# electrum/presto

Hardware: AMD Instinct MI355X
Metric: rows/s through operator pipeline, TPC-H Q1+Q6 SF100, 1/2/4/8 GPUs vs CPU ref (higher is better)
Workload: dtype f64

## Files before the change

presto_amd/csrc/fused_codegen.cpp:

```cpp
#include "decimal_host.hpp"
#include "fused_codegen.hpp"
#include "scan_kernels.hpp"

namespace pa {
namespace fused {

int range_entry_words(const Spec& s, const std::vector<ChannelLayout>& layout)
{
    int words = 1;
    for (int c = 0; c < s.n_in; c++) {
        if (!s.used_channel[c]) continue;
        words += 1 + (layout[c].type == PA_VARCHAR ? 1 : 0) + (layout[c].nullable ? 1 : 0);
    }
    return words;
}

static std::vector<ChannelLayout> extended_layout(const Spec& s, const std::vector<ChannelLayout>& layout)
{
    std::vector<ChannelLayout> ext(layout.begin(), layout.begin() + s.n_in);
    if (s.join) {
        for (size_t v = 0; v < s.join->build_cols.size(); v++) {
            ChannelLayout cl;
            cl.type = s.join->build_types[v];
            cl.nullable = (size_t)s.n_in + v < layout.size() ? layout[(size_t)s.n_in + v].nullable : true;
// ... 123 lines not shown
{
    if ((int)word_terms.size() <= w) word_terms.resize(w + 1);
    word_terms[w].push_back(term);
}

void FusedGen::group_keys()
{
    const std::vector<int>& gp = brow ? s.join->brow_group_proj : s.group_proj;
    std::ostringstream& kinner = brow ? key_os : inner;
    for (size_t gi = 0; gi < gp.size(); gi++) {
        const GenValue& kv = key_value(gp[gi]);
        const OwnedExpr& pe = s.proj[gp[gi]];
        KeyPart part;
        part.type = kv.type;
        std::string value;
        switch (kv.type) {
            case PA_BIGINT:
            case PA_DECIMAL:
                part.bits = 64;
                value = "(u64)" + kv.v;
                break;
            case PA_INTEGER:
            case PA_DATE:
                part.bits = 32;
                value = "(u64)(u32)(i32)" + kv.v;
                break;
            case PA_REAL:
                part.bits = 32;
                value = "(u64)pa_real_key_bits(" + kv.v + ")";
                break;
            case PA_BOOLEAN:
                part.bits = 1;
                value = "(" + kv.v + " ? 1ULL : 0ULL)";
                break;
            case PA_DOUBLE:
                part.bits = 64;
                value = "((" + kv.v + " == 0.0) ? 0ULL : ((" + kv.v + " != " + kv.v + ") ? 0x7ff8000000000000ULL : (u64)__double_as_longlong(" +
                        kv.v + ")))";
                break;
            case PA_VARCHAR: {
                int ch = pe.is_input_ref() ? pe.node(pe.root).channel : -1;
                if (ch >= 0 && ch < s.n_in && s.short_bound[ch] > 0) {
                    part.bound = s.short_bound[ch];
                    part.bits = 8 * part.bound + 4;
                    value = "(cs" + std::to_string(ch) + " | ((u64)" + kv.len + " << " + std::to_string(8 * part.bound) + "))";
                }
                else {
                    part.bits = 128;
                }
                break;
            }
            default:
                throw Error(PA_ERR_NOT_SUPPORTED, "group key type not supported on device");
        }
        std::string guard = kv.nullable() ? "(" + kv.n + ") ? 0ULL : " : "";
        if (part.bits == 128) {
            int sh;
            part.word = packer.place(64, &sh);
            int w2 = packer.place(64, &sh);
            PA_REQUIRE(w2 == part.word + 1, PA_ERR_NOT_SUPPORTED, "internal: long VARCHAR key words not adjacent");
            std::string id = "ks" + std::to_string(gi);
            kinner << "u64 " << id << "a = 0, " << id << "b = 0;\n";
            kinner << "if (" << (kv.nullable() ? "!" + kv.n : "true") << ") {\n";
            kinner << "  if (" << kv.len << " > 15) pa_raise(a.err, -3);\n";
            kinner << "  for (i32 b = 0; b < " << kv.len << " && b < 15; b++) {\n";
            kinner << "    if (b < 8) " << id << "a |= (u64)" << kv.v << "[b] << (8 * b); else " << id << "b |= (u64)" << kv.v
                  << "[b] << (8 * (b - 8));\n  }\n";
            kinner << "  " << id << "b |= (u64)" << kv.len << " << 56;\n}\n";
            add_term(part.word, id + "a");
            add_term(part.word + 1, id + "b");
        }
        else {
            part.word = packer.place(part.bits, &part.shift);
            add_term(part.word, "((" + guard + value + ") << " + std::to_string(part.shift) + ")");
        }
        if (kv.nullable()) {
            part.null_word = packer.place(1, &part.null_shift);
            add_term(part.null_word, "((" + kv.n + ") ? " + std::to_string(1ULL << part.null_shift) + "ULL : 0ULL)");
        }
        k.keys.push_back(part);
    }
    k.w = (int)packer.used.size();
    PA_REQUIRE(k.w <= 8, PA_ERR_NOT_SUPPORTED, "group key wider than 8 words");
}

int FusedGen::word(int kind, const std::string& cond, const std::string& val, const std::string& key)
{
    auto it = word_index.find(key);
    if (it != word_index.end()) return it->second;
    words.push_back({kind, cond, val});
    word_index[key] = (int)words.size() - 1;
    return (int)words.size() - 1;
}

std::string FusedGen::minmax_image(const GenValue& x, bool is_min)
{
    std::string img;
    switch (x.type) {
        case PA_BIGINT:
        case PA_INTEGER:
        case PA_DECIMAL:
        case PA_DATE: img = "pa_img_i64((i64)" + x.v + ")"; break;
        case PA_DOUBLE: img = "pa_img_f64(" + x.v + ")"; break;
        case PA_REAL: img = "pa_img_f64((double)" + x.v + ")"; break;
        case PA_BOOLEAN: img = "(" + x.v + " ? 1ULL : 0ULL)"; break;
        case PA_VARCHAR: img = "pa_img_str7(" + x.v + ", " + x.len + ", a.err)"; break;
        default: throw Error(PA_ERR_NOT_SUPPORTED, "min/max input type not supported on device");
    }
    return is_min ? "(~" + img + ")" : img;
}

std::string FusedGen::wtype(int w) const
{
    return words[w].kind == W_SUMF ? "double" : (words[w].kind == W_MAXU ? "u64" : "i64");
}

void FusedGen::accumulator_words()
{
    for (const auto& ag : s.aggs) {
        if (s.step == PA_STEP_FINAL) {
            const GenValue& c = proj_value(ag.input_channel);
            std::string ch = std::to_string(ag.input_channel);
            std::string ccond = c.nullable() ? "(!" + c.n + ")" : "true";
            int cw = word(W_CNT, ccond, c.v, "fcnt|" + ch);
            int vw = -1;
            if (ag.fn == PA_AGG_SUM || ag.fn == PA_AGG_AVG) {
                const GenValue& v = proj_value(ag.input_channel + 1);
                std::string vcond = v.nullable() ? "(" + ccond + " && !" + v.n + ")" : ccond;
                if (v.type == PA_LONG_DECIMAL) {
                    const int limbs = decimal_limbs_for_bits(128);
                    for (int l = 0; l < limbs; l++) {
                        const int w = word(W_SUMI, vcond, "pa_dec_limb(" + v.v + ", " + std::to_string(l) + ", " + std::to_string(limbs - 1) + ")", "fdec" + std::to_string(l) + "|" + ch);
                        if (l == 0) vw = w;
                        PA_REQUIRE(w == vw + l, PA_ERR_NOT_SUPPORTED, "internal: the limb words of a DECIMAL sum are not adjacent");
                    }
                    k.agg_words.emplace_back(cw, vw);
                    k.agg_limbs.resize(k.agg_words.size(), 0);
                    k.agg_limbs.back() = limbs;
                    continue;
                }
                vw = word(v.type == PA_DOUBLE ? W_SUMF : W_SUMI, vcond, v.v, "fsum|" + ch);
            }
            else if (ag.fn == PA_AGG_MIN || ag.fn == PA_AGG_MAX) {
                const GenValue& v = proj_value(ag.input_channel + 1);
                std::string vcond = v.nullable() ? "(" + ccond + " && !" + v.n + ")" : ccond;
                vw = word(W_MAXU, vcond, minmax_image(v, ag.fn == PA_AGG_MIN), std::string(ag.fn == PA_AGG_MIN ? "fmin|" : "fmax|") + ch);
            }
            k.agg_words.emplace_back(cw, vw);
            continue;
        }
        std::string cond = "true", ckey = "m" + std::to_string(ag.mask_channel);
        if (ag.mask_channel >= 0) {
            const GenValue& m = proj_value(ag.mask_channel);
            PA_REQUIRE(m.type == PA_BOOLEAN, PA_ERR_INVALID_ARGUMENT, "mask channel must be BOOLEAN");
            cond = m.nullable() ? "(!" + m.n + " && " + m.v + ")" : "(" + m.v + ")";
        }
        if (ag.fn == PA_AGG_COUNT_STAR) {
            k.agg_words.emplace_back(word(W_CNT, cond, "1", "cnt|*|" + ckey), -1);
            continue;
        }
        const GenValue& x = proj_value(ag.input_channel);
        std::string xkey = s.proj[ag.input_channel].fingerprint();
        std::string ccond = cond, cntkey = "cnt|*|" + ckey;
        if (x.nullable()) {
            ccond = "(" + cond + " && !" + x.n + ")";
            cntkey = "cnt|" + xkey + "|" + ckey;
        }
        const bool implicit_count = s.step == PA_STEP_SINGLE && !s.group_proj.empty() && ag.mask_channel < 0 && !x.nullable() &&
                                    (ag.fn == PA_AGG_SUM || ag.fn == PA_AGG_MIN || ag.fn == PA_AGG_MAX);
        int cw = implicit_count ? -1 : word(W_CNT, ccond, "1", cntkey);
        int vw = -1;
        if ((ag.fn == PA_AGG_SUM || ag.fn == PA_AGG_AVG) && (x.type == PA_DECIMAL || x.type == PA_LONG_DECIMAL)) {
            const int limbs = decimal_limbs_for_bits(std::min(x.type == PA_DECIMAL ? 64 : 128, decimal_bits_for_precision(PA_DECIMAL_PRECISION(x.param))));
            for (int l = 0; l < limbs; l++) {
                const int w = word(W_SUMI, ccond, "pa_dec_limb((i128)" + x.v + ", " + std::to_string(l) + ", " + std::to_string(limbs - 1) + ")",
                                   "dec" + std::to_string(l) + "/" + std::to_string(limbs) + "|" + xkey + "|" + ckey);
                if (l == 0) vw = w;
                PA_REQUIRE(w == vw + l, PA_ERR_NOT_SUPPORTED, "internal: the limb words of a DECIMAL sum are not adjacent");
            }
            k.agg_words.emplace_back(cw, vw);
            k.agg_limbs.resize(k.agg_words.size(), 0);
            k.agg_limbs.back() = limbs;
            continue;
        }
        if (ag.fn == PA_AGG_SUM && x.type != PA_DOUBLE && x.type != PA_REAL) {
            vw = word(W_SUMI, ccond, x.v, "sumi|" + xkey + "|" + ckey);
        }
        else if (ag.fn == PA_AGG_SUM || ag.fn == PA_AGG_AVG) {
            std::string v = x.type == PA_DOUBLE ? x.v : "((double)" + x.v + ")";
            vw = word(W_SUMF, ccond, v, std::string("sumf|") + (x.type == PA_DOUBLE ? "d|" : "i|") + xkey + "|" + ckey);
        }
        else if (ag.fn == PA_AGG_MIN || ag.fn == PA_AGG_MAX) {
            vw = word(W_MAXU, ccond, minmax_image(x, ag.fn == PA_AGG_MIN), std::string(ag.fn == PA_AGG_MIN ? "min|" : "max|") + xkey + "|" + ckey);
        }
        k.agg_words.emplace_back(cw, vw);
    }
    k.nw = (int)words.size();
    k.agg_limbs.resize(k.agg_words.size(), 0);
    PA_REQUIRE(k.nw > 0 || k.w > 0, PA_ERR_INVALID_ARGUMENT, "aggregation without aggregates and keys");
    if (k.nw == 0) {
        words.push_back({W_CNT, "true", "1"});
        k.nw = 1;
    }
    for (const auto& w : words) k.word_kind.push_back(w.kind);
}

void FusedGen::state_layout_id()
{
    std::vector<std::string> names(words.size(), "rows");
    for (const auto& kv : word_index) names[(size_t)kv.second] = kv.first;
    std::ostringstream id;
    for (const KeyPart& kp : k.keys) {
        id << kp.type << ',' << kp.word << ',' << kp.shift << ',' << kp.bits << ',' << kp.bound << ',' << kp.null_word << ',' << kp.null_shift << ';';
    }
    id << '#';
    for (size_t w = 0; w < words.size(); w++) id << words[w].kind << ':' << names[w] << ';';
    k.layout_id = id.str();
}

void FusedGen::row_function(const std::string& name)
{
    if (s.join) {
        probe_row_frames();
    }
    else {
        src << "__device__ __forceinline__ void " << name << "(const PaFusedArgs& a, PaAcc& acc, const bool live, const i32 row" << row_params(ri, layout) << ")\n{\n";
    }
    src << body.str();
    for (int w = 0; w < k.nw; w++) {
        src << "bool u" << w << " = false; " << (words[w].kind == W_SUMF ? "double" : (words[w].kind == W_MAXU ? "u64" : "i64")) << " x" << w << " = 0;\n";
    }
    if (k.w > 0) src << "u64 key[PA_KW];\n#pragma unroll\nfor (int i = 0; i < PA_KW; i++) key[i] = 0;\n";
    src << "if (sel) {\n" << build_loads.str() << inner.str();
    for (int w = 0; w < k.nw; w++) src << "u" << w << " = " << words[w].cond << "; x" << w << " = " << words[w].val << ";\n";
    if (brow) {
        src << "key[0] = (u64)(u32)jb;\n";
    }
    else {
        for (int i = 0; i < k.w; i++) {
            src << "key[" << i << "] = ";
            for (size_t t = 0; t < word_terms[i].size(); t++) src << (t ? " | " : "") << word_terms[i][t];
            src << ";\n";
        }
    }
    src << "}\n";
    if (variant == V_HASH) hash_accumulate_row();
    else if (variant == V_GLOBAL) global_accumulate_row();
    else if (variant == V_LDS) lds_accumulate_row();
    else if (brow) brow_accumulate_row();
    else table_accumulate_row();
    src << "}\n\n";
}

void FusedGen::emit_quad(const std::string (&args)[4])
{
    if (s.join) {
        probe_quad(args);
        return;
    }
    for (int r = 0; r < 4; r++) src << "        pa_row(a, acc, true, (i32)(4 * q + " << r << ")" << args[r] << ");\n";
}

void FusedGen::emit_kernel(const std::string& name, int mode)
{
    std::string occupancy;
    if (brow) {
        if (const char* e = getenv("PRESTO_AMD_BROW_WAVES")) occupancy = " __attribute__((amdgpu_waves_per_eu(" + std::to_string(atoi(e)) + ")))";
    }
    src << "extern \"C\" __global__ __launch_bounds__(" << B << ")" << occupancy << " void PA_K(" << name << ")(PaFusedArgs a)\n{\n";
    if (variant == V_GLOBAL) global_kernel_begin();
    else if (variant == V_LDS) lds_kernel_begin();
    else if (variant == V_LDSP) ldsp_kernel_begin();
    else if (variant == V_LDSH) ldsh_kernel_begin();
    else if (variant == V_HASH) hash_kernel_begin();
    else if (brow) brow_kernel_begin();
    else gt_kernel_begin();
    if (mode != 2 && mode != 3) emit_prologue(ri, layout, src);
    if (mode == 3) {
        ranges_loop();
    }
    else if (variant == V_GLOBAL) {
        global_thread_ids();
    }
    else {
        src << "    const i64 t = (i64)blockIdx.x * " << B << " + threadIdx.x, T = (i64)gridDim.x * " << B << ";\n";
    }
    if (mode == 3) {
    }
    else if (mode == 1) lds_head_loop();
    else if (mode == 2) lds_tail_loop();
    else if (variant == V_HASH) hash_tile_loop();
    else page_loop();
    if (variant == V_LDSP) ldsp_partition_loop();
    if (variant == V_GT || variant == V_LDSH) list_loops();
    if (variant == V_LDSH) ldsh_kernel_end();
    if (brow) brow_kernel_end();
    if (gt_like || brow || lds_table) table_counter_flush();
    if (variant == V_GLOBAL) global_kernel_end();
    else if (variant == V_LDS) lds_kernel_end();
    src << "}\n\n";
}

void FusedGen::ranges_loop()
{
    ColumnNames rn;
    rn.ranged = true;
    const int rw = range_entry_words(s, layout);
    src << "    const u32 bsw = (gridDim.x & 7u) == 0u ? (blockIdx.x & 7u) * (gridDim.x >> 3) + (blockIdx.x >> 3) : blockIdx.x;\n"
           "    for (i64 ri = bsw; ri < a.n_ranges; ri += gridDim.x) {\n"
           "      const u64* RT = a.ranges + (u64)ri * " << rw << "ULL;\n";
    int at = 0;
    for (int c = 0; c < s.n_in; c++) {
        if (!ri.used[c]) continue;
        src << "      const void* const RV" << c << " = (const void*)RT[" << at++ << "];\n";
        if (layout[c].type == PA_VARCHAR) src << "      const i32* const RO" << c << " = (const i32*)RT[" << at++ << "];\n";
        if (layout[c].nullable) src << "      const u8* const RNL" << c << " = (const u8*)RT[" << at++ << "];\n";
    }
    src << "      const i64 RN = (i64)(RT[" << at << "] & 0xffffffffULL);\n"
           "      const bool rvec = (RT[" << at << "] >> 32) != 0ULL;\n";
    {
        std::ostringstream pro;
        emit_prologue(ri, layout, pro, rn);
        src << pro.str();
    }
    if (variant == V_LDS) src << "      const i64 nq = rvec ? (RN >> 8) << 6 : 0;\n";
    else src << "      const i64 nq = rvec ? RN >> 2 : 0;\n";
    src << "      for (i64 q = threadIdx.x; q < nq; q += " << B << ") {\n";
    std::string rargs[4];
    emit_vector_loads(ri, layout, src, rargs, rn);
    emit_quad(rargs);
    src << "      }\n";
    if (variant == V_LDS) {
        src << "      for (i64 rb = nq << 2; rb < RN; rb += 64) {\n        const bool live = rb + threadIdx.x < RN;\n"
               "        const i64 r = live ? rb + threadIdx.x : RN - 1;\n        pa_row(a, acc, live, (i32)r" << scalar_args(ri, layout, rn) << ");\n      }\n";
    }
    else {
        src << "      for (i64 r = (nq << 2) + threadIdx.x; r < RN; r += " << B << ") {\n        pa_row(a, acc, true, (i32)r" << scalar_args(ri, layout, rn) << ");\n      }\n";
    }
    src << "    }\n";
}

void FusedGen::page_loop()
{
    std::string args[4];
    src << "    const i64 nq = a.vec ? (a.n >> 2) : 0;\n";
    const std::string tail_rows = "    for (i64 r = (nq << 2) + t; r < a.n; r += T) {\n        pa_row(a, acc, true, (i32)r" + scalar_args(ri, layout) + ");" + flush + "\n    }\n";
    bool two_loops = false;
    if (staged) {
        staged_page_loop();
        src << tail_rows;
        return;
    }
    if (brow) {
        int level = 3;
        if (const char* e = getenv("PRESTO_AMD_BROW_PIPE")) level = atoi(e);
        std::vector<VectorVar> vars;
        const bool can = level > 0 && s.join && vector_load_vars(ri, layout, vars);
        if (can && level < 3) {
            brow_pipelined_loop(level);
            src << tail_rows;
            return;
        }
        if (can) {
            src << "    if (a.jrank) {\n";
            brow_pipelined_loop(level);
            src << "    } else {\n";
            two_loops = true;
        }
        brow_wave_loop_head();
    }
    else {
// ... 17 lines not shown
```

presto_amd/csrc/fused_codegen.hpp:

```cpp
#pragma once

#include <functional>
#include <map>
#include <sstream>
#include <string>
#include <vector>

#include "fused_plan.hpp"
#include "rowgen.hpp"

namespace pa {
namespace fused {

struct KeyPacker {
    std::vector<int> used;
    int place(int bits, int* shift)
    {
        for (size_t w = 0; w < used.size(); w++) {
            if (used[w] + bits <= 64) {
                *shift = used[w];
                used[w] += bits;
                return (int)w;
            }
        }
        used.push_back(bits);
        *shift = 0;
        return (int)used.size() - 1;
    }
};

struct WordDef {
    int kind;
    std::string cond;
    std::string val;
};

struct FusedGen {
    FusedGen(const Spec& spec, const std::vector<ChannelLayout>& page_layout, int requested_variant);
    KernelInfo run();

    const Spec& s;
    const std::vector<ChannelLayout>& layout;
    int variant;
    bool ranged;
    KernelInfo k;
    RowInputs ri;
    std::vector<ChannelLayout> ext;
    RowCodegen gen;
    std::ostringstream body;
    std::ostringstream pre;
    std::ostringstream inner;
    std::ostringstream key_os;
    std::ostringstream build_loads;
    std::ostringstream src;
    std::map<int, GenValue> pv, kpv;
    KeyPacker packer;
    std::vector<std::vector<std::string>> word_terms;
    std::vector<WordDef> words;
    std::map<std::string, int> word_index;
    bool brow = false, lds_table = false, gt_like = false;
    bool staged = false;
    std::string lazy_params, lazy_names;
    int B = 256;
    std::string flush;

    const GenValue& proj_value(int j);
    const GenValue& key_value(int j);
    void add_term(int word, const std::string& term);
    int word(int kind, const std::string& cond, const std::string& val, const std::string& key);
    std::string minmax_image(const GenValue& x, bool is_min);
    std::string wtype(int w) const;
    void row_filter();
    void group_keys();
    void accumulator_words();
    void state_layout_id();
    void row_function(const std::string& name = "pa_row");
    void emit_quad(const std::string (&args)[4]);
    void emit_kernel(const std::string& name, int mode);
    void ranges_loop();
    void page_loop();
    void table_counter_flush();

    void global_declarations();
    void global_accumulate_row();
    void global_kernel_begin();
    void global_thread_ids();
    void global_kernel_end();
    void staged_row_functions();
    void staged_page_loop();

    void lds_check_capacity();
    void lds_declarations();
    void lds_accumulate_row();
    void lds_kernel_begin();
    void lds_head_loop();
    void lds_tail_loop();
    void lds_kernel_end();

    void lds_table_size();
    void lds_table_declarations();
    void lds_table_accumulate_begin();
    void ldsh_kernel_begin();
    void ldsh_kernel_end();

    void hash_declarations();
    void hash_accumulate_row();
    void hash_kernel_begin();
    void hash_tile_loop();
    void ldsp_kernel_begin();
    void ldsp_partition_loop();

    void gt_declarations();
    void table_accumulate();
    void gt_run_combining();
    void table_accumulate_row();
    void gt_kernel_begin();
    void list_loops();

    void probe_filter_and_key(const std::string& sel);
    void probe_occupancy_word();
    void probe_build_loads();
    std::string lazy_assign(const std::string& suffix, const std::string& row);
    std::string lazy_declare(const std::string& suffix);
    void probe_row_frames();
    void probe_row_composition();
    void probe_quad(const std::string (&args)[4]);
    void brow_declarations();
    void brow_accumulate_row();
    void brow_kernel_begin();
    void brow_wave_loop_head();
    bool brow_pipelined_loop(int level);
    void brow_kernel_end();
    void brow_keys_kernel();
};

}
}
```

presto_amd/csrc/fused_plan.hpp:

```cpp
#pragma once

#include <map>
#include <memory>
#include <string>
#include <vector>

#include "exprgen.hpp"
#include "join_source.hpp"
#include "operator.hpp"

namespace pa {
namespace fused {

constexpr int kMaxChannels = 32;
constexpr int kMaxBuildChannels = 8;

struct FusedArgs {
    const void* v[kMaxChannels];
    const int32_t* o[kMaxChannels];
    const uint8_t* nl[kMaxChannels];
    int64_t n;
    int32_t vec;
    int32_t pad;
    uint64_t* slab;
// ... 18 lines not shown
    uint64_t* sub_tag;
    uint64_t* sub_keys;
    uint64_t* sub_words;
    int32_t* sub_count;
    const int64_t* part_first;
    const void* jslots;
    const uint64_t* jbits;
    int64_t jmin;
    uint64_t jrange;
    uint32_t jmask;
    int32_t jrows;
    uint32_t jwrap;
    uint32_t jpad;
    const void* bv[kMaxBuildChannels];
    const uint8_t* bn[kMaxBuildChannels];
    const void* jrank;
    const int32_t* jrank_rows;
    const uint64_t* ranges;
    int64_t n_ranges;
};

enum Variant { V_GLOBAL = 0, V_LDS = 1, V_GT = 2, V_LDSH = 3, V_HASH = 4, V_LDSP = 5, V_BROW = 6, V_GLOBAL_R = 7, V_LDS_R = 8, V_GLOBAL_S = 9 };
constexpr int kMaxStages = 4;
constexpr int64_t kRangeRows = 8192, kRangeRowsLds = 4096;
enum WordKind { W_CNT = 0, W_SUMF = 1, W_SUMI = 2, W_MAXU = 3 };

constexpr int kLdsSlots = 8;

struct KeyPart {
    int32_t type = PA_BIGINT;
    int word = 0;
    int shift = 0;
    int bits = 64;
    int bound = 0;
    int null_word = -1;
    int null_shift = 0;
};

struct JoinStage {
    std::shared_ptr<LookupSourceImpl> ls;
    int key_proj = -1;
    std::vector<int> build_cols;
    std::vector<int32_t> build_types;
    std::vector<int> brow_group_proj;
};

struct Spec {
    std::shared_ptr<JoinStage> join;
    std::vector<bool> lazy_channel;
    std::vector<int32_t> conjuncts;
    std::vector<int> conjunct_begin;
    std::vector<int> channel_stage;
    int n_stages = 0;
    int n_in = 0;
    std::vector<int32_t> in_types, in_params;
    bool has_filter = false;
    OwnedExpr filter;
    std::vector<OwnedExpr> proj;
    std::vector<int> group_proj;
    int hash_channel = -1;
    std::vector<pa_aggregate> aggs;
    int expected_groups = 0;
    int64_t max_partial_memory = 0;
    int step = PA_STEP_SINGLE;
    int output_mem = PA_MEM_HOST;
    std::vector<bool> used_channel;
    std::vector<int> short_bound;
    std::vector<bool> interned;
    std::vector<bool> ranked;
    bool any_ranked() const
    {
        for (bool r : ranked) if (r) return true;
        return false;
    }
    bool derived(int c) const { return interned[c] || ranked[c]; }
};

struct KernelInfo {
    std::string source, entry;
    int variant = V_GLOBAL;
    bool ranged = false;
    std::vector<int> stage_bytes;
    int nw = 0, w = 0, c = 0, block = 256;
    int lc = 0;
    int occ_word = -1;
    uint64_t occ_empty = 0;
    std::vector<int32_t> word_kind;
    std::vector<std::pair<int, int>> agg_words;
    std::vector<int> agg_limbs;
    std::vector<KeyPart> keys;
    std::string layout_id;
};

struct LayoutChange {};

OwnedExpr input_ref_expr(int32_t channel, int32_t type);
Spec make_spec(const pa_filter_project_desc& fp, const pa_hash_aggregation_desc& ag, const pa_lookup_join_desc* jd = nullptr,
               pa_lookup_source* bridge = nullptr);
Spec make_spec(const pa_fused_aggregation_desc* d);
void finalize_spec(Spec& s);
void plan_stages(Spec& s);

int range_entry_words(const Spec& s, const std::vector<ChannelLayout>& layout);
KernelInfo generate(const Spec& s, const std::vector<ChannelLayout>& layout, int variant);

}
}
```

presto_amd/csrc/fused_tier_lds.cpp:

```cpp
#include "decimal_host.hpp"
#include "fused_codegen.hpp"
#include "scan_kernels.hpp"

namespace pa {
namespace fused {

void FusedGen::lds_check_capacity()
{
    PA_REQUIRE((size_t)k.nw * kLdsSlots * 64 * 8 <= 64 * 1024, PA_ERR_NOT_SUPPORTED, "too many accumulator words for the LDS variant");
}

void FusedGen::lds_declarations()
{
    src << "__shared__ u64 pa_accw[PA_NW * PA_C * 64];\n";
    src << "struct PaAcc { u64 tk[PA_C][PA_KW]; int tcount; u32 lane; };\n";
}

void FusedGen::lds_accumulate_row()
{
    src << "int g = -1;\nif (sel) {\n#pragma unroll\n  for (int s = 0; s < PA_C; s++) {\n    bool eq = s < acc.tcount;\n#pragma unroll\n"
           "    for (int w = 0; w < PA_KW; w++) eq = eq && (key[w] == acc.tk[s][w]);\n    if (eq) g = s;\n  }\n}\n";
    src << "u64 miss = __ballot(sel && g < 0);\nwhile (miss != 0ULL) {\n  const int src_lane = __builtin_amdgcn_readfirstlane(__ffsll((long long)miss) - 1);\n"
           "  u64 nk[PA_KW];\n#pragma unroll\n  for (int w = 0; w < PA_KW; w++) nk[w] = pa_readlane_u64(key[w], src_lane);\n"
           "  const int slot = acc.tcount;\n  if (slot < PA_C) {\n#pragma unroll\n    for (int s = 0; s < PA_C; s++) {\n      if (s == slot) {\n#pragma unroll\n"
           "        for (int w = 0; w < PA_KW; w++) acc.tk[s][w] = nk[w];\n      }\n    }\n    acc.tcount = slot + 1;\n  } else {\n    acc.tcount = PA_C + 1;\n  }\n"
           "  bool mine = sel && g == -1;\n#pragma unroll\n  for (int w = 0; w < PA_KW; w++) mine = mine && (key[w] == nk[w]);\n"
           "  if (mine) g = slot < PA_C ? slot : -2;\n  miss = __ballot(sel && g == -1);\n}\n";
    src << "if (sel) {\n  if (g >= 0) {\n";
    for (int w = 0; w < k.nw; w++) {
        std::string idx = "pa_accw[(" + std::to_string(w) + " * PA_C + g) * 64 + acc.lane]";
        if (words[w].kind == W_SUMF) {
            src << "    if (u" << w << ") __hip_atomic_fetch_add((double*)&" << idx << ", x" << w << ", __ATOMIC_RELAXED, __HIP_MEMORY_SCOPE_WORKGROUP);\n";
        }
        else if (words[w].kind == W_SUMI) {
            src << "    if (u" << w << ") { i64* p = (i64*)&" << idx << "; *p = pa_add_exact(*p, x" << w << ", a.err); }\n";
        }
        else if (words[w].kind == W_MAXU) {
            src << "    if (u" << w << ") { u64* p = &" << idx << "; if (x" << w << " > *p) *p = x" << w << "; }\n";
        }
        else {
            src << "    if (u" << w << ") __hip_atomic_fetch_add(&" << idx << ", " << (words[w].val == "1" ? std::string("1ULL") : "(u64)x" + std::to_string(w))
                << ", __ATOMIC_RELAXED, __HIP_MEMORY_SCOPE_WORKGROUP);\n";
        }
    }
    src << "  }\n}\n";
}

void FusedGen::lds_kernel_begin()
{
    src << "    for (int i = threadIdx.x; i < PA_NW * PA_C * 64; i += 64) pa_accw[i] = 0ULL;\n";
    src << "    __syncthreads();\n";
    src << "    PaAcc acc; acc.tcount = 0; acc.lane = threadIdx.x;\n";
    src << "#pragma unroll\n    for (int s = 0; s < PA_C; s++) {\n#pragma unroll\n        for (int w = 0; w < PA_KW; w++) acc.tk[s][w] = 0ULL;\n    }\n";
}

void FusedGen::lds_head_loop()
{
    std::string args[4];
    src << "    const i64 nq = a.n >> 2;  // the host passes a multiple of 256 rows\n";
    src << "    for (i64 q = t; q < nq; q += T) {\n";
    emit_vector_loads(ri, layout, src, args);
    emit_quad(args);
    src << "    }\n";
}

void FusedGen::lds_tail_loop()
{
    src << "    for (i64 rb = (i64)blockIdx.x * 64; rb < a.n; rb += T) {\n        const bool live = rb + threadIdx.x < a.n;\n"
           "        const i64 r = live ? rb + threadIdx.x : a.n - 1;\n        pa_row(a, acc, live, (i32)r" << scalar_args(ri, layout) << ");\n    }\n";
}

void FusedGen::lds_kernel_end()
{
    src << "    __syncthreads();\n";
    src << "    if (acc.tcount > PA_C && threadIdx.x == 0) atomicAdd((unsigned long long*)a.overflow_rows, 1ULL);\n";
    src << "    const u64 E = (u64)gridDim.x * PA_C;\n";
    src << "#pragma unroll\n    for (int i = 0; i < PA_C; i++) {\n        u64* e = a.slab + (u64)blockIdx.x * PA_C + i;\n";
    src << "        const bool occ = i < acc.tcount;\n        if (threadIdx.x == 0) e[0] = occ ? 1ULL : 0ULL;\n        if (occ) {\n";
    src << "#pragma unroll\n            for (int w = 0; w < PA_KW; w++) { if (threadIdx.x == 0) e[(u64)(1 + w) * E] = acc.tk[i][w]; }\n";
    for (int w = 0; w < k.nw; w++) {
        std::string idx = "pa_accw[(" + std::to_string(w) + " * PA_C + i) * 64 + threadIdx.x]";
        std::string dst = "e[(u64)(1 + PA_KW + " + std::to_string(w) + ") * E]";
        if (words[w].kind == W_SUMF) src << "            { double v = pa_wave_sum_f64(__longlong_as_double((i64)" << idx << ")); if (threadIdx.x == 0) " << dst << " = (u64)__double_as_longlong(v); }\n";
        else if (words[w].kind == W_SUMI) src << "            { i64 v = pa_wave_sum_i64_exact((i64)" << idx << ", a.err); if (threadIdx.x == 0) " << dst << " = (u64)v; }\n";
        else if (words[w].kind == W_MAXU) src << "            { u64 v = pa_wave_max_u64(" << idx << "); if (threadIdx.x == 0) " << dst << " = v; }\n";
        else src << "            { i64 v = pa_wave_sum_i64((i64)" << idx << "); if (threadIdx.x == 0) " << dst << " = (u64)v; }\n";
    }
    src << "        }\n    }\n";
}

}
}
```

presto_amd/csrc/op_fused.cpp:

```cpp
#include <algorithm>
#include <cstring>
#include <sstream>

#include "op_fused.hpp"

namespace pa {
namespace fused_op {

FusedAggregationOperator::FusedAggregationOperator(const pa_fused_aggregation_desc* d)
    : FusedAggregationOperator(make_spec(d), d->aggregation.stream ? d->aggregation.stream : d->filter_project.stream)
{
}

FusedAggregationOperator::FusedAggregationOperator(Spec spec, void* stream) : spec_(std::move(spec)), stream_(stream)
{
    require_device();
    nullable_seen_.assign(spec_.n_in, false);
    out_partial_ = spec_.step == PA_STEP_PARTIAL;
    {
        std::ostringstream f;
        for (int c = 0; c < spec_.n_in; c++) f << spec_.in_types[c] << ',' << spec_.in_params[c] << ';';
        f << '|' << (spec_.has_filter ? spec_.filter.fingerprint() : std::string("-")) << '|';
        for (const auto& p : spec_.proj) f << p.fingerprint() << '#';
        f << '|';
        for (int g : spec_.group_proj) f << g << ',';
        f << '|' << spec_.hash_channel << '|' << spec_.step << '|';
        for (const auto& a : spec_.aggs) f << a.fn << ',' << a.input_channel << ',' << a.mask_channel << ',' << a.input_type << ';';
        if (spec_.join) {
            f << "|join:" << spec_.join->key_proj << ':';
            for (int32_t t : spec_.join->build_types) f << t << ',';
            f << ':';
            for (int j : spec_.join->brow_group_proj) f << j << ',';
        }
        plan_fingerprint_ = f.str();
    }
    grouped_ = !spec_.group_proj.empty();
    mode_ = grouped_ ? (spec_.expected_groups > (1 << 20) ? V_GT : V_LDS) : V_GLOBAL;
    if (spec_.any_ranked() && grouped_) mode_ = V_GT;
    cus_ = device_cu_count();
    ctl_ = static_cast<int32_t*>(ctl_buf_.ensure(64));
    PA_HIP(hipMemsetAsync(ctl_, 0, 64, stream_.get()));
    h_ctl_ = static_cast<int32_t*>(h_ctl_buf_.ensure(256));
    memset(h_ctl_, 0, 256);
}

FusedAggregationOperator::~FusedAggregationOperator()
{
    (void)hipStreamSynchronize(stream_.get());
    if (lds_.merge_stream) pool_stream_release(lds_.merge_stream);
    release_everything();
    for (hipEvent_t e : release_events_) (void)hipEventDestroy(e);
    for (int b = 0; b < 2; b++) {
        if (arena_[b].table_event) (void)hipEventDestroy(arena_[b].table_event);
        if (arena_[b].vtable_event) (void)hipEventDestroy(arena_[b].vtable_event);
        if (lds_.ev_main[b]) (void)hipEventDestroy(lds_.ev_main[b]);
        if (lds_.ev_merge[b]) (void)hipEventDestroy(lds_.ev_merge[b]);
    }
    for (RangeTable& t : range_table_) {
        if (t.event) (void)hipEventDestroy(t.event);
    }
}

bool FusedAggregationOperator::set_output_topn(int64_t n, const int32_t* channels, const int32_t* orders, int32_t count)
{
    if (n <= 0 || count <= 0 || !grouped_ || out_partial_ || spec_.step == PA_STEP_PARTIAL) return false;
    topn_hint_.n = n;
    topn_hint_.channels.assign(channels, channels + count);
    topn_hint_.orders.assign(orders, orders + count);
    return true;
}

bool FusedAggregationOperator::retry_parked()
{
    if (!parked_) return true;
    if (!pool_has_room(parked_need_)) return false;
    parked_ = false;
    pa_page page = parked_page_;
    page.columns = parked_cols_.data();
    take_page(&page);
    return !parked_;
}

void FusedAggregationOperator::take_page(const pa_page* page)
{
    const uint64_t launched = timer.begun();
    try {
        if (next_) {
            next_->add_input(page);
            return;
        }
        cur_rel_set_ = (page->flags & PA_PAGE_RETAINED) != 0 && page->release != nullptr;
        cur_rel_ = Release{page->release, page->release_ctx};
        if (gather_small_page(page)) return;
        flush_pending();
        if (next_) {
            cur_rel_set_ = false;
            next_->add_input(page);
            return;
        }
        process_page(page, page_stays(page) && page->mem == PA_MEM_DEVICE);
        if (cur_rel_set_) {
            std::vector<Release> rel{cur_rel_};
            cur_rel_set_ = false;
            release_checkpoint(std::move(rel), true);
        }
    }
    catch (const PoolExhausted& e) {
        if (!page_stays(page) || timer.begun() != launched || is_combiner_) throw;
        parked_page_ = *page;
        if (!cur_rel_set_) parked_page_.flags &= ~PA_PAGE_RETAINED;
        cur_rel_set_ = false;
        parked_cols_.assign(page->columns, page->columns + page->channel_count);
        parked_need_ = e.bytes;
        parked_ = true;
    }
}
// ... 312 lines not shown
```

presto_amd/csrc/rowgen.cpp:

```cpp
#include "rowgen.hpp"

namespace pa {

std::string row_params(const RowInputs& s, const std::vector<ChannelLayout>& layout)
{
    std::ostringstream p;
    for (int c = 0; c < s.n_in; c++) {
        if (!s.used[c]) continue;
        p << ", " << RowCodegen::ctype(layout[c].type) << " c" << c;
        if (layout[c].type == PA_VARCHAR) p << ", i32 cl" << c;
        if (s.short_bound[c] > 0) p << ", u64 cs" << c;
        if (layout[c].nullable) p << ", bool cn" << c;
    }
    return p.str();
}

std::string row_param_names(const RowInputs& s, const std::vector<ChannelLayout>& layout)
{
    std::ostringstream p;
    for (int c = 0; c < s.n_in; c++) {
        if (!s.used[c]) continue;
        p << ", c" << c;
        if (layout[c].type == PA_VARCHAR) p << ", cl" << c;
        if (s.short_bound[c] > 0) p << ", cs" << c;
        if (layout[c].nullable) p << ", cn" << c;
    }
    return p.str();
}

void emit_prologue(const RowInputs& s, const std::vector<ChannelLayout>& layout, std::ostringstream& o, const ColumnNames& nm)
{
    for (int c = 0; c < s.n_in; c++) {
        if (!s.used[c] || layout[c].type != PA_VARCHAR || s.short_bound[c] != 1) continue;
        o << "    const i32 P" << c << " = " << nm.n() << " > 0 ? " << nm.o(c) << "[0] : 0;\n";
        o << "    const i64 PB" << c << " = " << nm.n() << " > 0 ? (i64)" << nm.o(c) << "[" << nm.n() << "] - P" << c << " : 0;\n";
        o << "    const bool U" << c << " = PB" << c << " == (i64)" << nm.n() << ";\n";
    }
}

void emit_vector_loads(const RowInputs& s, const std::vector<ChannelLayout>& layout, std::ostringstream& o, std::string args[4], const ColumnNames& nm)
{
    static const char* xyzw[4] = {"x", "y", "z", "w"};
    std::ostringstream mid, post;
    for (int c = 0; c < s.n_in; c++) {
        if (!s.used[c]) continue;
        const std::string C = std::to_string(c), V = nm.v(c), O = nm.o(c), NL = nm.nl(c);
        switch (layout[c].type) {
            case PA_BIGINT:
            case PA_DECIMAL:
                o << "        pa_i64x2 A" << C << " = ((const pa_i64x2*)" << V << ")[2 * q], B" << C << " = ((const pa_i64x2*)" << V
                  << ")[2 * q + 1];\n";
                for (int r = 0; r < 4; r++) args[r] += ", " + std::string(r < 2 ? "A" : "B") + C + "." + xyzw[r & 1];
                break;
            case PA_LONG_DECIMAL:
                for (int r = 0; r < 4; r++) {
                    o << "        pa_i64x2 L" << C << r << " = ((const pa_i64x2*)" << V << ")[4 * q + " << r << "];\n";
                    args[r] += ", pa_ld_from(L" + C + std::to_string(r) + ".x, L" + C + std::to_string(r) + ".y)";
                }
                break;
            case PA_DOUBLE:
                o << "        pa_f64x2 A" << C << " = ((const pa_f64x2*)" << V << ")[2 * q], B" << C << " = ((const pa_f64x2*)" << V
                  << ")[2 * q + 1];\n";
                for (int r = 0; r < 4; r++) args[r] += ", " + std::string(r < 2 ? "A" : "B") + C + "." + xyzw[r & 1];
                break;
            case PA_INTEGER:
            case PA_DATE:
                o << "        pa_i32x4 A" << C << " = ((const pa_i32x4*)" << V << ")[q];\n";
                for (int r = 0; r < 4; r++) args[r] += ", (i64)A" + C + "." + xyzw[r];
                break;
            case PA_REAL:
                o << "        pa_f32x4 A" << C << " = ((const pa_f32x4*)" << V << ")[q];\n";
                for (int r = 0; r < 4; r++) args[r] += ", A" + C + "." + xyzw[r];
                break;
            case PA_BOOLEAN:
                o << "        u32 A" << C << " = ((const u32*)" << V << ")[q];\n";
                for (int r = 0; r < 4; r++) args[r] += ", ((A" + C + " >> " + std::to_string(8 * r) + ") & 0xffu) != 0u";
                break;
            case PA_VARCHAR: {
                const std::string load_offsets = "O" + C + " = ((const pa_i32x4*)" + O + ")[q]; E" + C + " = " + O + "[4 * q + 4];";
                if (s.short_bound[c] == 1) {
                    mid << "        pa_i32x4 O" << C << "; i32 E" << C << ";\n        if (U" << C << " && (K" << C << " & 0x80808080u) == 0u) {\n"
                        << "            const i32 b = P" << C << " + (i32)(4 * q);\n            O" << C << ".x = b; O" << C << ".y = b + 1; O" << C
                        << ".z = b + 2; O" << C << ".w = b + 3; E" << C << " = b + 4;\n        } else {\n            " << load_offsets << "\n        }\n";
                }
                else {
                    o << "        pa_i32x4 O" << C << " = ((const pa_i32x4*)" << O << ")[q]; i32 E" << C << " = " << O << "[4 * q + 4];\n";
                }
                std::string lo[4], len[4];
                for (int r = 0; r < 4; r++) {
                    lo[r] = "O" + C + "." + xyzw[r];
                    len[r] = (r < 3 ? "O" + C + "." + xyzw[r + 1] : "E" + C) + " - " + lo[r];
                }
                if (s.short_bound[c] > 0) {
                    post << "        u64 S" << C << "0, S" << C << "1, S" << C << "2, S" << C << "3;\n";
                    if (s.short_bound[c] == 1) {
                        o << "        u32 K" << C << " = 0u; if (4 * q + 4 <= PB" << C << ") __builtin_memcpy(&K" << C << ", (const u8*)" << V
                          << " + P" << C << " + 4 * q, 4);\n";
                        post << "        if (E" << C << " - " << lo[0] << " == 4) {\n            u32 pk = K" << C << ";\n            if (" << lo[0]
                             << " != P" << C << " + (i32)(4 * q) || 4 * q + 4 > PB" << C << ") __builtin_memcpy(&pk, (const u8*)" << V << " + "
                             << lo[0] << ", 4);\n";
                        for (int r = 0; r < 4; r++) post << "            S" << C << r << " = (pk >> " << 8 * r << ") & 0xffu;\n";
                        post << "        } else {\n";
                    }
                    else {
                        post << "        {\n";
                    }
                    for (int r = 0; r < 4; r++) {
                        post << "            S" << C << r << " = pa_short_bytes((const u8*)" << V << " + " << lo[r] << ", " << len[r] << ", "
                             << s.short_bound[c] << ", a.err);\n";
                    }
                    post << "        }\n";
                }
                for (int r = 0; r < 4; r++) {
                    args[r] += ", (const u8*)" + V + " + " + lo[r] + ", " + len[r];
                    if (s.short_bound[c] > 0) args[r] += ", S" + C + std::to_string(r);
                }
                break;
            }
            default:
                throw Error(PA_ERR_NOT_SUPPORTED, "column type not supported on device");
        }
        if (layout[c].nullable) {
            o << "        u32 N" << C << " = " << NL << " ? ((const u32*)" << NL << ")[q] : 0u;\n";
            for (int r = 0; r < 4; r++) args[r] += ", ((N" + C + " >> " + std::to_string(8 * r) + ") & 0xffu) != 0u";
        }
    }
    o << mid.str() << post.str();
}

std::string VectorVar::load(const std::string& q) const
{
    const std::string idx = per_quad == 2 ? "2 * (" + q + ")" + (half ? " + 1" : "") : "(" + q + ")";
    const std::string ld = "((const " + type + "*)" + array + ")[" + idx + "]";
    return maybe_null ? "(" + array + " ? " + ld + " : 0u)" : ld;
}

bool vector_load_vars(const RowInputs& s, const std::vector<ChannelLayout>& layout, std::vector<VectorVar>& vars, const ColumnNames& nm)
{
    vars.clear();
    for (int c = 0; c < s.n_in; c++) {
        if (!s.used[c]) continue;
        const std::string C = std::to_string(c);
        const size_t first = vars.size();
        switch (layout[c].type) {
            case PA_BIGINT:
            case PA_DECIMAL:
                vars.push_back(VectorVar{"pa_i64x2", "A" + C, nm.v(c), 2, 0, false});
                vars.push_back(VectorVar{"pa_i64x2", "B" + C, nm.v(c), 2, 1, false});
                break;
            case PA_DOUBLE:
                vars.push_back(VectorVar{"pa_f64x2", "A" + C, nm.v(c), 2, 0, false});
                vars.push_back(VectorVar{"pa_f64x2", "B" + C, nm.v(c), 2, 1, false});
                break;
            case PA_INTEGER:
            case PA_DATE: vars.push_back(VectorVar{"pa_i32x4", "A" + C, nm.v(c), 1, 0, false}); break;
            case PA_REAL: vars.push_back(VectorVar{"pa_f32x4", "A" + C, nm.v(c), 1, 0, false}); break;
            case PA_BOOLEAN: vars.push_back(VectorVar{"u32", "A" + C, nm.v(c), 1, 0, false}); break;
            default: return false;
        }
        if (layout[c].nullable) vars.push_back(VectorVar{"u32", "N" + C, nm.nl(c), 1, 0, true});
        for (size_t i = first; i < vars.size(); i++) vars[i].channel = c;
    }
    return true;
}

std::string vector_var_args(const RowInputs& s, const std::vector<ChannelLayout>& layout, const std::string& P, int r)
{
    std::string a;
    for (int c = 0; c < s.n_in; c++) {
        if (s.used[c]) a += vector_var_channel_args(layout, P, r, c);
    }
    return a;
}

std::string vector_var_channel_args(const std::vector<ChannelLayout>& layout, const std::string& P, int r, int c)
{
    static const char* xyzw[4] = {"x", "y", "z", "w"};
    std::string a;
    const std::string C = std::to_string(c);
    switch (layout[c].type) {
        case PA_BIGINT:
        case PA_DECIMAL:
        case PA_DOUBLE: a += ", " + P + std::string(r < 2 ? "A" : "B") + C + "." + xyzw[r & 1]; break;
        case PA_INTEGER:
        case PA_DATE: a += ", (i64)" + P + "A" + C + "." + xyzw[r]; break;
        case PA_REAL: a += ", " + P + "A" + C + "." + xyzw[r]; break;
        case PA_BOOLEAN: a += ", ((" + P + "A" + C + " >> " + std::to_string(8 * r) + ") & 0xffu) != 0u"; break;
        default: throw Error(PA_ERR_NOT_SUPPORTED, "column type not supported on device");
    }
    if (layout[c].nullable) a += ", ((" + P + "N" + C + " >> " + std::to_string(8 * r) + ") & 0xffu) != 0u";
    return a;
}

std::string scalar_loads(const RowInputs& s, const std::vector<ChannelLayout>& layout, const std::string& row, const std::string& suffix, std::ostringstream& decl,
                         const ColumnNames& nm)
{
    std::string a;
    for (int c = 0; c < s.n_in; c++) {
        if (!s.used[c]) continue;
        const std::string C = std::to_string(c), V = nm.v(c), O = nm.o(c), NL = nm.nl(c), L = "l" + C + suffix;
        switch (layout[c].type) {
            case PA_BIGINT:
            case PA_DECIMAL: decl << "const i64 " << L << " = ((const i64*)" << V << ")[" << row << "]; "; a += ", " + L; break;
            case PA_LONG_DECIMAL: decl << "const i128 " << L << " = pa_ld_read((const u64*)" << V << " + 2 * (" << row << ")); "; a += ", " + L; break;
            case PA_DOUBLE: decl << "const double " << L << " = ((const double*)" << V << ")[" << row << "]; "; a += ", " + L; break;
            case PA_INTEGER:
// ... 49 lines not shown
```

presto_amd/csrc/rowgen.hpp:

```cpp
#pragma once

#include <sstream>
#include <string>
#include <vector>

#include "exprgen.hpp"

namespace pa {

struct RowInputs {
    int n_in = 0;
    std::vector<bool> used;
    std::vector<int> short_bound;
};

struct ColumnNames {
    bool ranged = false;
    std::string v(int c) const { return ranged ? "RV" + std::to_string(c) : "a.v[" + std::to_string(c) + "]"; }
    std::string o(int c) const { return ranged ? "RO" + std::to_string(c) : "a.o[" + std::to_string(c) + "]"; }
    std::string nl(int c) const { return ranged ? "RNL" + std::to_string(c) : "a.nl[" + std::to_string(c) + "]"; }
    std::string n() const { return ranged ? "RN" : "a.n"; }
};

std::string row_params(const RowInputs& s, const std::vector<ChannelLayout>& layout);
std::string row_param_names(const RowInputs& s, const std::vector<ChannelLayout>& layout);
void emit_prologue(const RowInputs& s, const std::vector<ChannelLayout>& layout, std::ostringstream& o, const ColumnNames& names = ColumnNames());
void emit_vector_loads(const RowInputs& s, const std::vector<ChannelLayout>& layout, std::ostringstream& o, std::string args[4],
                       const ColumnNames& names = ColumnNames());
struct VectorVar {
    std::string type, name, array;
    int per_quad;
    int half;
    bool maybe_null;
    int channel = -1;
    std::string load(const std::string& q) const;
};
bool vector_load_vars(const RowInputs& s, const std::vector<ChannelLayout>& layout, std::vector<VectorVar>& vars, const ColumnNames& names = ColumnNames());
std::string vector_var_args(const RowInputs& s, const std::vector<ChannelLayout>& layout, const std::string& prefix, int r);
std::string vector_var_channel_args(const std::vector<ChannelLayout>& layout, const std::string& prefix, int r, int c);
std::string scalar_loads(const RowInputs& s, const std::vector<ChannelLayout>& layout, const std::string& row, const std::string& suffix,
                         std::ostringstream& decl, const ColumnNames& names = ColumnNames());
std::string scalar_args(const RowInputs& s, const std::vector<ChannelLayout>& layout, const ColumnNames& names = ColumnNames());

}
```

Measured before the change: 203.4 billion.

## Prefetch next quad loads in LDS head loop and pack narrow group keys

For the LDS aggregation tier, group keys that fit in 31 bits are held as a single u32 instead of an array of u64 words, which shrinks per-thread key state and the compare loop when finding a group. The LDS head loop also gains a software-pipelined form: it loads the next grid-stride quad's columns into registers before processing the current one, hiding global memory latency behind compute. The prefetch path is on by default, can be turned off with an environment variable, and is folded into the plan fingerprint. The cost is higher register pressure from the double-buffered loads, and on varchar slow paths the code inserts explicit waitcnt drains.

Measured after the change: 210.7 billion, median of 6. 1.04x the previous value.

```diff
diff --git a/presto_amd/csrc/fused_codegen.cpp b/presto_amd/csrc/fused_codegen.cpp
--- a/presto_amd/csrc/fused_codegen.cpp
+++ b/presto_amd/csrc/fused_codegen.cpp
@@ -229,6 +229,7 @@
     }
     k.w = (int)packer.used.size();
     PA_REQUIRE(k.w <= 8, PA_ERR_NOT_SUPPORTED, "group key wider than 8 words");
+    k.packed_key = !brow && k.w == 1 && packer.used[0] <= 31;
 }
 
 int FusedGen::word(int kind, const std::string& cond, const std::string& val, const std::string& key)
@@ -377,7 +378,9 @@
     for (int w = 0; w < k.nw; w++) {
         src << "bool u" << w << " = false; " << (words[w].kind == W_SUMF ? "double" : (words[w].kind == W_MAXU ? "u64" : "i64")) << " x" << w << " = 0;\n";
     }
-    if (k.w > 0) src << "u64 key[PA_KW];\n#pragma unroll\nfor (int i = 0; i < PA_KW; i++) key[i] = 0;\n";
+    const bool key32 = variant == V_LDS && k.packed_key;
+    if (key32) src << "u32 key = 0u;\n";
+    else if (k.w > 0) src << "u64 key[PA_KW];\n#pragma unroll\nfor (int i = 0; i < PA_KW; i++) key[i] = 0;\n";
     src << "if (sel) {\n" << build_loads.str() << inner.str();
     for (int w = 0; w < k.nw; w++) src << "u" << w << " = " << words[w].cond << "; x" << w << " = " << words[w].val << ";\n";
     if (brow) {
@@ -385,9 +388,9 @@
     }
     else {
         for (int i = 0; i < k.w; i++) {
-            src << "key[" << i << "] = ";
+            src << (key32 ? "key = (u32)(" : "key[" + std::to_string(i) + "] = ");
             for (size_t t = 0; t < word_terms[i].size(); t++) src << (t ? " | " : "") << word_terms[i][t];
-            src << ";\n";
+            src << (key32 ? ");\n" : ";\n");
         }
     }
     src << "}\n";
@@ -434,6 +437,7 @@
     }
     if (mode == 3) {
     }
+    else if (mode == 1 && k.packed_key && lds_pipe_level() > 0) lds_head_loop_ahead();
     else if (mode == 1) lds_head_loop();
     else if (mode == 2) lds_tail_loop();
     else if (variant == V_HASH) hash_tile_loop();
diff --git a/presto_amd/csrc/fused_codegen.hpp b/presto_amd/csrc/fused_codegen.hpp
--- a/presto_amd/csrc/fused_codegen.hpp
+++ b/presto_amd/csrc/fused_codegen.hpp
@@ -91,9 +91,12 @@
 
     void lds_check_capacity();
     void lds_declarations();
+    void lds_find_group();
+    void lds_find_group_packed();
     void lds_accumulate_row();
     void lds_kernel_begin();
     void lds_head_loop();
+    void lds_head_loop_ahead();
     void lds_tail_loop();
     void lds_kernel_end();
 
diff --git a/presto_amd/csrc/fused_plan.hpp b/presto_amd/csrc/fused_plan.hpp
--- a/presto_amd/csrc/fused_plan.hpp
+++ b/presto_amd/csrc/fused_plan.hpp
@@ -124,6 +124,7 @@
     bool ranged = false;
     std::vector<int> stage_bytes;
     int nw = 0, w = 0, c = 0, block = 256;
+    bool packed_key = false;
     int lc = 0;
     int occ_word = -1;
     uint64_t occ_empty = 0;
@@ -145,6 +146,7 @@
 
 int range_entry_words(const Spec& s, const std::vector<ChannelLayout>& layout);
 KernelInfo generate(const Spec& s, const std::vector<ChannelLayout>& layout, int variant);
+int lds_pipe_level();
 
 }
 }
diff --git a/presto_amd/csrc/fused_tier_lds.cpp b/presto_amd/csrc/fused_tier_lds.cpp
--- a/presto_amd/csrc/fused_tier_lds.cpp
+++ b/presto_amd/csrc/fused_tier_lds.cpp
@@ -1,9 +1,17 @@
+#include <cstdlib>
+
 #include "decimal_host.hpp"
 #include "fused_codegen.hpp"
 #include "scan_kernels.hpp"
 
 namespace pa {
 namespace fused {
+
+int lds_pipe_level()
+{
+    const char* e = getenv("PRESTO_AMD_LDS_PIPE");
+    return e ? atoi(e) : 1;
+}
 
 void FusedGen::lds_check_capacity()
 {
@@ -13,10 +21,21 @@
 void FusedGen::lds_declarations()
 {
     src << "__shared__ u64 pa_accw[PA_NW * PA_C * 64];\n";
-    src << "struct PaAcc { u64 tk[PA_C][PA_KW]; int tcount; u32 lane; };\n";
+    if (k.packed_key) src << "struct PaAcc { u32 tk[PA_C]; int tcount; u32 lane; };\n";
+    else src << "struct PaAcc { u64 tk[PA_C][PA_KW]; int tcount; u32 lane; };\n";
 }
 
-void FusedGen::lds_accumulate_row()
+void FusedGen::lds_find_group_packed()
+{
+    src << "int g = -1;\nif (sel) {\n#pragma unroll\n  for (int s = 0; s < PA_C; s++) {\n    if (key == acc.tk[s]) g = s;\n  }\n}\n";
+    src << "u64 miss = __ballot(sel && g < 0);\nwhile (miss != 0ULL) {\n  const int src_lane = __builtin_amdgcn_readfirstlane(__ffsll((long long)miss) - 1);\n"
+           "  const u32 nk = (u32)__builtin_amdgcn_readlane((int)key, src_lane);\n"
+           "  const int slot = acc.tcount;\n  if (slot < PA_C) {\n#pragma unroll\n    for (int s = 0; s < PA_C; s++) {\n      if (s == slot) acc.tk[s] = nk;\n    }\n"
+           "    acc.tcount = slot + 1;\n  } else {\n    acc.tcount = PA_C + 1;\n  }\n"
+           "  if (sel && g == -1 && key == nk) g = slot < PA_C ? slot : -2;\n  miss = __ballot(sel && g == -1);\n}\n";
+}
+
+void FusedGen::lds_find_group()
 {
     src << "int g = -1;\nif (sel) {\n#pragma unroll\n  for (int s = 0; s < PA_C; s++) {\n    bool eq = s < acc.tcount;\n#pragma unroll\n"
            "    for (int w = 0; w < PA_KW; w++) eq = eq && (key[w] == acc.tk[s][w]);\n    if (eq) g = s;\n  }\n}\n";
@@ -26,6 +45,12 @@
            "        for (int w = 0; w < PA_KW; w++) acc.tk[s][w] = nk[w];\n      }\n    }\n    acc.tcount = slot + 1;\n  } else {\n    acc.tcount = PA_C + 1;\n  }\n"
            "  bool mine = sel && g == -1;\n#pragma unroll\n  for (int w = 0; w < PA_KW; w++) mine = mine && (key[w] == nk[w]);\n"
            "  if (mine) g = slot < PA_C ? slot : -2;\n  miss = __ballot(sel && g == -1);\n}\n";
+}
+
+void FusedGen::lds_accumulate_row()
+{
+    if (k.packed_key) lds_find_group_packed();
+    else lds_find_group();
     src << "if (sel) {\n  if (g >= 0) {\n";
     for (int w = 0; w < k.nw; w++) {
         std::string idx = "pa_accw[(" + std::to_string(w) + " * PA_C + g) * 64 + acc.lane]";
@@ -51,6 +76,10 @@
     src << "    for (int i = threadIdx.x; i < PA_NW * PA_C * 64; i += 64) pa_accw[i] = 0ULL;\n";
     src << "    __syncthreads();\n";
     src << "    PaAcc acc; acc.tcount = 0; acc.lane = threadIdx.x;\n";
+    if (k.packed_key) {
+        src << "#pragma unroll\n    for (int s = 0; s < PA_C; s++) acc.tk[s] = 0xFFFFFFFFu;\n";
+        return;
+    }
     src << "#pragma unroll\n    for (int s = 0; s < PA_C; s++) {\n#pragma unroll\n        for (int w = 0; w < PA_KW; w++) acc.tk[s][w] = 0ULL;\n    }\n";
 }
 
@@ -60,6 +89,27 @@
     src << "    const i64 nq = a.n >> 2;  // the host passes a multiple of 256 rows\n";
     src << "    for (i64 q = t; q < nq; q += T) {\n";
     emit_vector_loads(ri, layout, src, args);
+    emit_quad(args);
+    src << "    }\n";
+}
+
+void FusedGen::lds_head_loop_ahead()
+{
+    std::string args[4];
+    std::vector<QuadLoad> loads;
+    std::ostringstream rest;
+    emit_vector_loads(ri, layout, rest, args, ColumnNames(), &loads);
+    src << "    const i64 nq = a.n >> 2;  // the host passes a multiple of 256 rows\n";
+    for (const QuadLoad& l : loads) src << "    " << l.type << " n" << l.name << " = {};\n";
+    src << "    if (t < nq) {\n";
+    for (const QuadLoad& l : loads) src << "        " << l.into("n" + l.name, "t") << "\n";
+    src << "    }\n";
+    src << "    for (i64 q = t; q < nq; q += T) {\n";
+    for (const QuadLoad& l : loads) src << "        const " << l.type << " " << l.name << " = n" << l.name << ";\n";
+    src << "        const i64 qn = q + T;\n        if (qn < nq) {\n";
+    for (const QuadLoad& l : loads) src << "            " << l.into("n" + l.name, "qn") << "\n";
+    src << "        }\n";
+    src << rest.str();
     emit_quad(args);
     src << "    }\n";
 }
@@ -77,7 +127,8 @@
     src << "    const u64 E = (u64)gridDim.x * PA_C;\n";
     src << "#pragma unroll\n    for (int i = 0; i < PA_C; i++) {\n        u64* e = a.slab + (u64)blockIdx.x * PA_C + i;\n";
     src << "        const bool occ = i < acc.tcount;\n        if (threadIdx.x == 0) e[0] = occ ? 1ULL : 0ULL;\n        if (occ) {\n";
-    src << "#pragma unroll\n            for (int w = 0; w < PA_KW; w++) { if (threadIdx.x == 0) e[(u64)(1 + w) * E] = acc.tk[i][w]; }\n";
+    if (k.packed_key) src << "            if (threadIdx.x == 0) e[E] = (u64)acc.tk[i];  // (the slab's key word is what it is for every key)\n";
+    else src << "#pragma unroll\n            for (int w = 0; w < PA_KW; w++) { if (threadIdx.x == 0) e[(u64)(1 + w) * E] = acc.tk[i][w]; }\n";
     for (int w = 0; w < k.nw; w++) {
         std::string idx = "pa_accw[(" + std::to_string(w) + " * PA_C + i) * 64 + threadIdx.x]";
         std::string dst = "e[(u64)(1 + PA_KW + " + std::to_string(w) + ") * E]";
diff --git a/presto_amd/csrc/op_fused.cpp b/presto_amd/csrc/op_fused.cpp
--- a/presto_amd/csrc/op_fused.cpp
+++ b/presto_amd/csrc/op_fused.cpp
@@ -32,6 +32,7 @@
             f << ':';
             for (int j : spec_.join->brow_group_proj) f << j << ',';
         }
+        f << "|lds_pipe:" << lds_pipe_level();
         plan_fingerprint_ = f.str();
     }
     grouped_ = !spec_.group_proj.empty();
diff --git a/presto_amd/csrc/rowgen.cpp b/presto_amd/csrc/rowgen.cpp
--- a/presto_amd/csrc/rowgen.cpp
+++ b/presto_amd/csrc/rowgen.cpp
@@ -38,42 +38,64 @@
     }
 }
 
-void emit_vector_loads(const RowInputs& s, const std::vector<ChannelLayout>& layout, std::ostringstream& o, std::string args[4], const ColumnNames& nm)
+std::string QuadLoad::into(const std::string& dst, const std::string& q) const
+{
+    std::string out;
+    for (size_t i = 0; i < stmt.size(); i++) {
+        if (stmt[i] == '@' && i + 1 < stmt.size() && (stmt[i + 1] == 'd' || stmt[i + 1] == 'q')) out += stmt[++i] == 'd' ? dst : "(" + q + ")";
+        else out += stmt[i];
+    }
+    return out;
+}
+
+void emit_vector_loads(const RowInputs& s, const std::vector<ChannelLayout>& layout, std::ostringstream& o, std::string args[4], const ColumnNames& nm,
+                       std::vector<QuadLoad>* ahead)
 {
     static const char* xyzw[4] = {"x", "y", "z", "w"};
     std::ostringstream mid, post;
+    const std::string drain = ahead ? " __builtin_amdgcn_s_waitcnt(0x0F70);" : "";
+    auto halves = [&](const std::string& type, const std::string& C, const std::string& V) {
+        ahead->push_back({type, "A" + C, "@d = ((const " + type + "*)" + V + ")[2 * @q];"});
+        ahead->push_back({type, "B" + C, "@d = ((const " + type + "*)" + V + ")[2 * @q + 1];"});
+    };
     for (int c = 0; c < s.n_in; c++) {
         if (!s.used[c]) continue;
         const std::string C = std::to_string(c), V = nm.v(c), O = nm.o(c), NL = nm.nl(c);
         switch (layout[c].type) {
             case PA_BIGINT:
             case PA_DECIMAL:
-                o << "        pa_i64x2 A" << C << " = ((const pa_i64x2*)" << V << ")[2 * q], B" << C << " = ((const pa_i64x2*)" << V
-                  << ")[2 * q + 1];\n";
+                if (ahead) halves("pa_i64x2", C, V);
+                else o << "        pa_i64x2 A" << C << " = ((const pa_i64x2*)" << V << ")[2 * q], B" << C << " = ((const pa_i64x2*)" << V
+                       << ")[2 * q + 1];\n";
                 for (int r = 0; r < 4; r++) args[r] += ", " + std::string(r < 2 ? "A" : "B") + C + "." + xyzw[r & 1];
                 break;
             case PA_LONG_DECIMAL:
                 for (int r = 0; r < 4; r++) {
-                    o << "        pa_i64x2 L" << C << r << " = ((const pa_i64x2*)" << V << ")[4 * q + " << r << "];\n";
+                    if (ahead) ahead->push_back({"pa_i64x2", "L" + C + std::to_string(r), "@d = ((const pa_i64x2*)" + V + ")[4 * @q + " + std::to_string(r) + "];"});
+                    else o << "        pa_i64x2 L" << C << r << " = ((const pa_i64x2*)" << V << ")[4 * q + " << r << "];\n";
                     args[r] += ", pa_ld_from(L" + C + std::to_string(r) + ".x, L" + C + std::to_string(r) + ".y)";
                 }
                 break;
             case PA_DOUBLE:
-                o << "        pa_f64x2 A" << C << " = ((const pa_f64x2*)" << V << ")[2 * q], B" << C << " = ((const pa_f64x2*)" << V
-                  << ")[2 * q + 1];\n";
+                if (ahead) halves("pa_f64x2", C, V);
+                else o << "        pa_f64x2 A" << C << " = ((const pa_f64x2*)" << V << ")[2 * q], B" << C << " = ((const pa_f64x2*)" << V
+                       << ")[2 * q + 1];\n";
                 for (int r = 0; r < 4; r++) args[r] += ", " + std::string(r < 2 ? "A" : "B") + C + "." + xyzw[r & 1];
                 break;
             case PA_INTEGER:
             case PA_DATE:
-                o << "        pa_i32x4 A" << C << " = ((const pa_i32x4*)" << V << ")[q];\n";
+                if (ahead) ahead->push_back({"pa_i32x4", "A" + C, "@d = ((const pa_i32x4*)" + V + ")[@q];"});
+                else o << "        pa_i32x4 A" << C << " = ((const pa_i32x4*)" << V << ")[q];\n";
                 for (int r = 0; r < 4; r++) args[r] += ", (i64)A" + C + "." + xyzw[r];
                 break;
             case PA_REAL:
-                o << "        pa_f32x4 A" << C << " = ((const pa_f32x4*)" << V << ")[q];\n";
+                if (ahead) ahead->push_back({"pa_f32x4", "A" + C, "@d = ((const pa_f32x4*)" + V + ")[@q];"});
+                else o << "        pa_f32x4 A" << C << " = ((const pa_f32x4*)" << V << ")[q];\n";
                 for (int r = 0; r < 4; r++) args[r] += ", A" + C + "." + xyzw[r];
                 break;
             case PA_BOOLEAN:
-                o << "        u32 A" << C << " = ((const u32*)" << V << ")[q];\n";
+                if (ahead) ahead->push_back({"u32", "A" + C, "@d = ((const u32*)" + V + ")[@q];"});
+                else o << "        u32 A" << C << " = ((const u32*)" << V << ")[q];\n";
                 for (int r = 0; r < 4; r++) args[r] += ", ((A" + C + " >> " + std::to_string(8 * r) + ") & 0xffu) != 0u";
                 break;
             case PA_VARCHAR: {
@@ -81,7 +103,11 @@
                 if (s.short_bound[c] == 1) {
                     mid << "        pa_i32x4 O" << C << "; i32 E" << C << ";\n        if (U" << C << " && (K" << C << " & 0x80808080u) == 0u) {\n"
                         << "            const i32 b = P" << C << " + (i32)(4 * q);\n            O" << C << ".x = b; O" << C << ".y = b + 1; O" << C
-                        << ".z = b + 2; O" << C << ".w = b + 3; E" << C << " = b + 4;\n        } else {\n            " << load_offsets << "\n        }\n";
+                        << ".z = b + 2; O" << C << ".w = b + 3; E" << C << " = b + 4;\n        } else {\n            " << load_offsets << drain << "\n        }\n";
+                }
+                else if (ahead) {
+                    ahead->push_back({"pa_i32x4", "O" + C, "@d = ((const pa_i32x4*)" + O + ")[@q];"});
+                    ahead->push_back({"i32", "E" + C, "@d = " + O + "[4 * @q + 4];"});
                 }
                 else {
                     o << "        pa_i32x4 O" << C << " = ((const pa_i32x4*)" << O << ")[q]; i32 E" << C << " = " << O << "[4 * q + 4];\n";
@@ -94,11 +120,12 @@
                 if (s.short_bound[c] > 0) {
                     post << "        u64 S" << C << "0, S" << C << "1, S" << C << "2, S" << C << "3;\n";
                     if (s.short_bound[c] == 1) {
-                        o << "        u32 K" << C << " = 0u; if (4 * q + 4 <= PB" << C << ") __builtin_memcpy(&K" << C << ", (const u8*)" << V
-                          << " + P" << C << " + 4 * q, 4);\n";
+                        if (ahead) ahead->push_back({"u32", "K" + C, "@d = 0u; if (4 * @q + 4 <= PB" + C + ") __builtin_memcpy(&@d, (const u8*)" + V + " + P" + C + " + 4 * @q, 4);"});
+                        else o << "        u32 K" << C << " = 0u; if (4 * q + 4 <= PB" << C << ") __builtin_memcpy(&K" << C << ", (const u8*)" << V
+                               << " + P" << C << " + 4 * q, 4);\n";
                         post << "        if (E" << C << " - " << lo[0] << " == 4) {\n            u32 pk = K" << C << ";\n            if (" << lo[0]
-                             << " != P" << C << " + (i32)(4 * q) || 4 * q + 4 > PB" << C << ") __builtin_memcpy(&pk, (const u8*)" << V << " + "
-                             << lo[0] << ", 4);\n";
+                             << " != P" << C << " + (i32)(4 * q) || 4 * q + 4 > PB" << C << ") " << (ahead ? "{ " : "") << "__builtin_memcpy(&pk, (const u8*)" << V
+                             << " + " << lo[0] << ", 4);" << (ahead ? drain + " }" : "") << "\n";
                         for (int r = 0; r < 4; r++) post << "            S" << C << r << " = (pk >> " << 8 * r << ") & 0xffu;\n";
                         post << "        } else {\n";
                     }
@@ -109,6 +136,7 @@
                         post << "            S" << C << r << " = pa_short_bytes((const u8*)" << V << " + " << lo[r] << ", " << len[r] << ", "
                              << s.short_bound[c] << ", a.err);\n";
                     }
+                    if (ahead && s.short_bound[c] == 1) post << "           " << drain << "\n";
                     post << "        }\n";
                 }
                 for (int r = 0; r < 4; r++) {
@@ -121,7 +149,8 @@
                 throw Error(PA_ERR_NOT_SUPPORTED, "column type not supported on device");
         }
         if (layout[c].nullable) {
-            o << "        u32 N" << C << " = " << NL << " ? ((const u32*)" << NL << ")[q] : 0u;\n";
+            if (ahead) ahead->push_back({"u32", "N" + C, "@d = " + NL + " ? ((const u32*)" + NL + ")[@q] : 0u;"});
+            else o << "        u32 N" << C << " = " << NL << " ? ((const u32*)" << NL << ")[q] : 0u;\n";
             for (int r = 0; r < 4; r++) args[r] += ", ((N" + C + " >> " + std::to_string(8 * r) + ") & 0xffu) != 0u";
         }
     }
diff --git a/presto_amd/csrc/rowgen.hpp b/presto_amd/csrc/rowgen.hpp
--- a/presto_amd/csrc/rowgen.hpp
+++ b/presto_amd/csrc/rowgen.hpp
@@ -25,8 +25,12 @@
 std::string row_params(const RowInputs& s, const std::vector<ChannelLayout>& layout);
 std::string row_param_names(const RowInputs& s, const std::vector<ChannelLayout>& layout);
 void emit_prologue(const RowInputs& s, const std::vector<ChannelLayout>& layout, std::ostringstream& o, const ColumnNames& names = ColumnNames());
+struct QuadLoad {
+    std::string type, name, stmt;
+    std::string into(const std::string& dst, const std::string& q) const;
+};
 void emit_vector_loads(const RowInputs& s, const std::vector<ChannelLayout>& layout, std::ostringstream& o, std::string args[4],
-                       const ColumnNames& names = ColumnNames());
+                       const ColumnNames& names = ColumnNames(), std::vector<QuadLoad>* ahead = nullptr);
 struct VectorVar {
     std::string type, name, array;
     int per_quad;
```
